# medvedevgroup/TwoPaCo

Measured on AMD Instinct MI355X. Metric: kmers_hashed_per_sec, higher is better.
Workload: dtype u64

## Files before the change

### twopaco_amd/csrc/tpc_capi.hip

```cpp
#include "tpc_ctx.h"

namespace tpch {

int fail(tpc_ctx *c, int code, const char *fmt, ...)
{
    char buf[512];
    va_list ap;
    va_start(ap, fmt);
    vsnprintf(buf, sizeof buf, fmt, ap);
    va_end(ap);
    if (c) c->err = buf;
    return code;
}





TpcLaunch make_launch(const tpc_ctx *c)
{
    TpcLaunch a;
    a.P = c->P; a.tab = c->tab; a.bases = c->bases; a.nmask = c->nmask; a.n_text = c->n_text;
    a.n_tiles = c->n_tiles; a.filter = c->filter; a.stream = c->stream;
    a.stat_kernel = c->stat_kernel;
// ... 242 lines not shown
}

extern "C" {

int tpc_ctx_create(int device, tpc_ctx **out)
{
    if (!out) return -1;
    *out = nullptr;
    int n = 0;
    if (hipGetDeviceCount(&n) != hipSuccess || n <= 0) return -2;
    if (device < 0 || device >= n) return -3;
    if (hipSetDevice(device) != hipSuccess) return -4;
    tpc_ctx *c = new tpc_ctx();
    c->device = device;
    c->dbg_ovf = getenv("TPC_DEBUG_OVF") != nullptr; c->dbg_phases = getenv("TPC_PROFILE_PHASES") != nullptr; c->dbg_timing = getenv("TWOPACO_TIMING") != nullptr; c->no_lean = TpcEnv::get().no_lean;
    if (const char *e = getenv("TPC_SHARD_TIGHT")) c->opt_shard_tight = atoi(e) ? 1 : 0;
    if (hipStreamCreate(&c->stream) != hipSuccess) { delete c; return -5; }
    for (int i = 0; i < TPC_K_COUNT; i++) {
        if (hipEventCreate(&c->ev0[i]) != hipSuccess || hipEventCreate(&c->ev1[i]) != hipSuccess) { delete c; return -5; }
    }
    if (hipMalloc((void **)&c->tab, sizeof c->tab_host) != hipSuccess ||
        hipMalloc((void **)&c->counters, 8 * sizeof(unsigned long long)) != hipSuccess ||
        hipMalloc((void **)&c->route_scratch, 128 * sizeof(unsigned long long)) != hipSuccess) { delete c; return -6; }
    *out = c;
    return 0;
}

void tpc_ctx_destroy(tpc_ctx *c)
{
    if (!c) return;
    (void)hipSetDevice(c->device);
    (void)hipStreamSynchronize(c->stream);
    void *ptrs[] = { c->tab, c->bases_alloc, c->nmask_alloc, c->filter, c->rmask, c->mask, c->marks, c->block_sums, c->table,
                     c->keys, c->idtab, c->emit_id, c->stream_buf, c->counters, c->route_scratch, c->sh_off, c->scan_blocks, c->sort_scratch, c->seg.name, c->seg.first, c->seg.ev[0], c->seg.ev[1], c->seg.ev[2],
                     c->seg.rec, c->seg.amb, c->text_plan.off, c->text_plan.piece, c->text_names, c->text_win };
    for (void *p : ptrs) if (p) (void)hipFree(p);
    stream_part_release(c);
    colors_drop(c);
    links_drop(c);
    anchors_drop(c);
    edges_drop(c);
    for (void *p : c->pbuf) if (p) (void)hipFree(p);
    for (void *p : c->ikeep) if (p) (void)hipFree(p);
    if (c->periodic) (void)hipFree(c->periodic);
    if (c->cmb_base) (void)hipFree(c->cmb_base);
    if (c->cmb_cur) (void)hipFree(c->cmb_cur);
    if (c->ikeep_ovf) (void)hipFree(c->ikeep_ovf);
    if (c->iovf_cnt) (void)hipFree(c->iovf_cnt);
    if (c->iovf_off) (void)hipFree(c->iovf_off);
    for (int i = 0; i < TPC_K_COUNT; i++) { if (c->ev0[i]) (void)hipEventDestroy(c->ev0[i]); if (c->ev1[i]) (void)hipEventDestroy(c->ev1[i]); }
    if (c->stream2) (void)hipStreamDestroy(c->stream2);
    if (c->stream) (void)hipStreamDestroy(c->stream);
    delete c;
}

const char *tpc_last_error(const tpc_ctx *c) { return c ? c->err.c_str() : "null context"; }

int tpc_set_option(tpc_ctx *c, const char *name, int64_t value)
{
    if (!c || !name) return -1;
    if (!strcmp(name, "insert_test_first")) { c->opt_test_first = value != 0; return 0; }
    if (!strcmp(name, "insert_mode")) { c->opt_insert_mode = (int)value; return 0; }
    if (!strcmp(name, "slice_bits")) { c->opt_slice_bits = (int)value; return 0; }
    if (!strcmp(name, "query_mode")) { c->opt_query_mode = (int)value; return 0; }
    if (!strcmp(name, "part_budget_bytes")) { c->opt_part_budget = value; return 0; }
    if (!strcmp(name, "part_levels")) { c->opt_part_levels = (int)value; return 0; }
    if (!strcmp(name, "shard_tight_regions")) { c->opt_shard_tight = value ? 1 : 0; c->sh_have[0] = c->sh_have[1] = false; return 0; }
    if (!strcmp(name, "part_min_tiles")) { c->opt_part_min_tiles = value < 1 ? 1 : value; return 0; }
    if (!strcmp(name, "verify_marks")) { c->opt_verify_marks = value != 0; return 0; }
    if (!strcmp(name, "mark_bucket_bits")) { tpc_test_mark_bucket_bits = (int)value; return 0; }
    if (!strcmp(name, "mark_region_cap")) { tpc_test_mark_region_cap = (int)value; return 0; }
    if (!strcmp(name, "mark_slice_bits")) { tpc_test_mark_slice_bits = (int)value; return 0; }
    if (!strcmp(name, "qhash_pushes")) { tpc_opt_qhash_pushes = value == 8 ? 8 : 6; return 0; }
    if (!strcmp(name, "qhash_roll_scalars")) { tpc_opt_qhash_roll = value != 0; return 0; }
    if (!strcmp(name, "qhash_seed_scalars")) { tpc_opt_qhash_seed = value != 0; return 0; }
    if (!strcmp(name, "fuse_apply_lookup")) { c->opt_fuse = value != 0; return 0; }
    if (!strcmp(name, "test_q6_pb2")) { tpc_test_q6_pb2 = (int)value; return 0; }
    if (!strcmp(name, "insert_entry_fmt")) { tpc_test_insert_p3 = value == 3; return 0; }
    if (!strcmp(name, "shard_periodic_skip")) { c->opt_shard_periodic = value != 0; return 0; }
    if (!strcmp(name, "periodic_skip")) { c->opt_periodic = value != 0; if (!value) c->periodic_valid = false; return 0; }
    if (!strcmp(name, "test_tight_pinch")) { tpc_test_tight_pinch = (int)value; c->sh_have[0] = c->sh_have[1] = false; return 0; }
    if (!strcmp(name, "test_sched_cap")) { tpc_test_sched_cap = value > 0 ? (uint32_t)value : 0; return 0; }
    if (!strcmp(name, "test_mask_scan")) { tpc_test_mask_scan = value == 1 || value == 2 ? (int)value : 0; return 0; }
    if (!strcmp(name, "text_window")) { c->opt_text_window = value != 0; return 0; }
    if (!strcmp(name, "replicate_filter")) { c->opt_replicate = value != 0; return 0; }
    if (!strcmp(name, "test_force_anyq")) { tpc_test_force_anyq = value != 0; return 0; }
    if (!strcmp(name, "test_sketch_grid")) { tpc_test_sketch_grid = value > 0 ? (int)value : 0; return 0; }
    if (!strcmp(name, "test_links_slots_log2")) { c->opt_links_slots_log2 = (int)std::max<int64_t>(-1, std::min<int64_t>(value, 64)); return 0; }
    if (!strcmp(name, "test_edges_slots_log2")) { c->opt_edges_slots_log2 = (int)std::max<int64_t>(-1, std::min<int64_t>(value, 64)); return 0; }
    if (!strcmp(name, "test_edges_hash_bits")) { c->opt_edges_hash_bits = (int)std::max<int64_t>(-1, std::min<int64_t>(value, 65)); return 0; }
    if (!strcmp(name, "test_locate_grid")) { c->opt_locate_grid = value > 0 ? (int)std::min<int64_t>(value, 1 << 20) : 0; return 0; }
    if (!strcmp(name, "test_distances_chunk_words")) { c->opt_distances_chunk_words = (int)std::max<int64_t>(-1, std::min<int64_t>(value, 1 << 20)); return 0; }
    if (!strcmp(name, "test_components_step_limit")) { c->opt_components_step_limit = (int)std::max<int64_t>(-1, std::min<int64_t>(value, 0x7FFFFFFF)); return 0; }
    if (!strcmp(name, "test_fail_mallocs")) { tpc_test_fail_mallocs.store(value > 0 ? (int)value : 0); return 0; }
    return fail(c, -1, "unknown option %s", name);
}

int tpc_preload(int device)
{
    if (hipSetDevice(device) != hipSuccess) { (void)hipGetLastError(); return -10; }
    const bool timing = getenv("TWOPACO_TIMING") != nullptr;
    int (*const warm[4])() = { tpc_warm_partition, tpc_warm_qpartition, tpc_warm_pass2, tpc_warm_stream };
    const char *const name[4] = { "partition", "qpartition", "pass2", "stream" };
    for (int i = 0; i < 4; i++) {
        const auto t0 = std::chrono::steady_clock::now();
        if (warm[i]() != 0) return -10;
        if (timing) fprintf(stderr, "[timing]     code object %s: %.1f ms\n", name[i], std::chrono::duration<double, std::milli>(std::chrono::steady_clock::now() - t0).count());
    }
    return 0;
}

int tpc_warmup(tpc_ctx *c)
{
    if (!c) return -1;
    return tpc_preload(c->device);
}

int64_t tpc_get_stat(const tpc_ctx *c, const char *name)
{
    if (!c || !name) return -1;
    if (!strcmp(name, "insert_path")) return c->stat_path[0];
    if (!strcmp(name, "query_path")) return c->stat_path[1];
    if (!strcmp(name, "insert_entry_fmt")) return c->stat_fmt[0];
    if (!strcmp(name, "query_entry_fmt")) return c->stat_fmt[1];
    if (!strcmp(name, "insert_hash_kernel")) return c->stat_kernel[0];
    if (!strcmp(name, "query_hash_kernel")) return c->stat_kernel[1];
    if (!strcmp(name, "query_verify_kernel")) return c->stat_kernel[2];
    if (!strcmp(name, "query_hash_form")) return c->stat_kernel[3];
    if (!strcmp(name, "query_hash_seed")) return c->stat_kernel[4];
    if (!strcmp(name, "split_kernel")) return c->stat_split[0];
    if (!strcmp(name, "split_phases")) return c->stat_split[1];
    if (!strcmp(name, "query_hash_seed_maxk")) return TPC_QSEED_MAXK;
    if (!strcmp(name, "query_mark_path")) return c->stat_mark_path;
    if (!strcmp(name, "query_mark_fallback")) return c->stat_mark_fallback;
    if (!strcmp(name, "insert_batches")) return c->stat_batches[0];
    if (!strcmp(name, "query_batches")) return c->stat_batches[1];
    if (!strcmp(name, "query_tiles_per_batch")) return c->stat_q_plan[0];
    if (!strcmp(name, "query_b1")) return c->stat_q_plan[1];
    if (!strcmp(name, "query_b2")) return c->stat_q_plan[2];
    if (!strcmp(name, "query_begun")) return c->stat_q_begun;
    if (!strcmp(name, "filter2_retries")) return c->stat_filter2_retries;
    if (!strcmp(name, "aggregate_retries")) return c->stat_aggregate_retries;
    if (!strcmp(name, "filter2_counted")) return c->stat_filter2_counted;
    if (!strcmp(name, "fused_lookups")) return c->stat_fused;
    if (!strcmp(name, "query_overflow_entries")) return c->stat_query_overflow;
    if (!strcmp(name, "insert_overflow_entries")) return c->stat_insert_overflow;
    if (!strcmp(name, "periodic_skip")) return c->periodic_valid ? 1 : 0;
    if (!strcmp(name, "pbuf_releases")) return c->stat_pbuf_releases;
    if (!strcmp(name, "distances_tile")) return TPC_DISTANCES_TILE;
    if (!strcmp(name, "text_words")) return (int64_t)(c->text_w1 - c->text_w0);
    if (!strcmp(name, "text_word_begin")) return (int64_t)c->text_w0;
    if (!strcmp(name, "text_word_end")) return (int64_t)c->text_w1;
    if (!strcmp(name, "periodic_any_query")) return c->periodic_valid && c->periodic_any_q ? 1 : 0;
    if (!strcmp(name, "periodic_any_insert")) return c->periodic_valid && c->periodic_any_i ? 1 : 0;
    if (!strcmp(name, "text_write_us")) return c->text_write_us;
    if (!strcmp(name, "text_wait_us")) return c->text_wait_us;
    if (!strcmp(name, "text_window_bytes")) return c->text_window_bytes;
    if (!strcmp(name, "device_free_bytes") || !strcmp(name, "device_total_bytes")) {
        size_t free_b = 0, total_b = 0;
        if (hipSetDevice(c->device) != hipSuccess || hipMemGetInfo(&free_b, &total_b) != hipSuccess) { (void)hipGetLastError(); return -1; }
        return (int64_t)(name[7] == 'f' ? free_b : total_b);
    }
    if (!strcmp(name, "mask_scan_form")) return tpc_stat_mask_scan_form.load(std::memory_order_relaxed);
    if (!strcmp(name, "round_marks")) return c->marks_valid ? (int64_t)c->n_marks : -1;
    return -1;
}

// ... 673 lines not shown
```

### twopaco_amd/csrc/tpc_capi_pass2.hip

```cpp
#include "tpc_ctx.h"

namespace {
int pass2_filter_impl(tpc_ctx *c, const uint64_t *fmarks, uint64_t n_fmarks, bool external, uint64_t abundance, uint64_t *n_true, uint64_t *n_false, uint64_t *table_size,
                      bool records = false, bool aggregated = false);
inline bool aggregated_counted(uint64_t abundance) { return abundance < (1ull << 40); }
}

int tpc_pass2_filter(tpc_ctx *c, uint64_t abundance, uint64_t *n_true, uint64_t *n_false, uint64_t *table_size)
{
    return pass2_filter_impl(c, nullptr, 0, false, abundance, n_true, n_false, table_size);
}

int tpc_pass2_marks(tpc_ctx *c, uint64_t *n_marks)
{
    if (!c || !c->have_params || !c->bases || !n_marks) return fail(c, -1, "set_params and seq_upload first");
    HIPCHK(c, hipSetDevice(c->device));
    int rc = compact_mask(c, c->rmask);
    if (rc) return rc;
    c->marks_valid = true;
    *n_marks = c->n_marks;
    return 0;
}

int tpc_pass2_mark_owners(tpc_ctx *c, uint32_t world, uint64_t *pos_dev, int32_t *owner_dev)
// ... 164 lines not shown
                            : tpc_launch_scan2_write(a, c->C, marks, c->table, cap, abundance, counted, c->scan_blocks, c->keys + c->n_keys * c->C))
                    return fail(c, -1, "scan2 launch failed");
                c->n_keys += tp;
            }
        }
        if (!too_full) break;
        if (cap >= full) return fail(c, -1, "exact-filter table overflow at full size");
        cap = full;
        c->stat_filter2_retries++;
    }
    if (c->rounds_done == 0) {
        HIPCHK(c, hipMemcpyAsync(c->mask, c->rmask, c->n_words_alloc * sizeof(uint32_t), hipMemcpyDeviceToDevice, c->stream));
    } else {
        tpc_launch_mask_or(c->stream, c->mask, c->rmask, c->n_words_alloc);
        c->mask_dirty = true;
    }
    c->rounds_done++;
    c->finalized = false;
    HIPCHK(c, hipGetLastError());
    HIPCHK(c, hipStreamSynchronize(c->stream));
    if (n_true) *n_true = tp;
    if (n_false) *n_false = used - tp;
    if (table_size) *table_size = used;
    return 0;
}

}

int tpc_junctions_finalize(tpc_ctx *c, uint64_t *n_junctions)
{
    if (!c || !c->have_params) return fail(c, -1, "set_params first");
    HIPCHK(c, hipSetDevice(c->device));
    {
        Timed t(c, TPC_K_SORT);
        int rc = tpc_launch_sort_keys(c->stream, c->C, c->P.k, c->keys, c->n_keys, &c->sort_scratch, &c->sort_scratch_bytes);
        if (rc) return fail(c, rc, "key sort failed (%d)", rc);
        uint64_t cap = 1024;
        while (cap < 2 * c->n_keys + 2) cap <<= 1;
        const size_t slot_bytes = c->C == 1 ? 16 : 4;
        if (cap * slot_bytes > c->idtab_bytes) {
            if (c->idtab) (void)hipFree(c->idtab);
            c->idtab = nullptr;
            c->idtab_bytes = 0;
            HIPCHK(c, dev_malloc(c, (void **)&c->idtab, cap * slot_bytes));
            c->idtab_bytes = cap * slot_bytes;
        }
        c->idtab_cap = cap;
        HIPCHK(c, hipMemsetAsync(c->idtab, 0, cap * slot_bytes, c->stream));
        if (c->n_keys >= 0xFFFFFFFFull) return fail(c, -1, "too many junctions for the 32-bit id index");
        tpc_launch_idtab_build(c->stream, c->C, c->keys, c->n_keys, c->idtab, cap);
    }
    HIPCHK(c, hipGetLastError());
    HIPCHK(c, hipStreamSynchronize(c->stream));
    c->finalized = true;
    c->keys_host.clear();
    if (n_junctions) *n_junctions = c->n_keys;
    return 0;
}

int tpc_key_words(const tpc_ctx *c) { return c ? c->C : 0; }

int tpc_junction_keys(tpc_ctx *c, uint64_t *keys_host)
{
    if (!c || !c->finalized) return fail(c, -1, "junctions_finalize first");
    HIPCHK(c, hipSetDevice(c->device));
    if (c->n_keys) HIPCHK(c, hipMemcpy(keys_host, c->keys, c->n_keys * c->C * sizeof(uint64_t), hipMemcpyDeviceToHost));
    return 0;
}

int tpc_junction_keys_raw(tpc_ctx *c, uint64_t *keys_host, uint64_t *n)
{
    if (!c || !n) return -1;
    HIPCHK(c, hipSetDevice(c->device));
    *n = c->n_keys;
    if (keys_host && c->n_keys) {
        HIPCHK(c, hipStreamSynchronize(c->stream));
        HIPCHK(c, hipMemcpy(keys_host, c->keys, c->n_keys * c->C * sizeof(uint64_t), hipMemcpyDeviceToHost));
    }
    return 0;
}

int tpc_junction_keys_set(tpc_ctx *c, const uint64_t *keys_host, uint64_t n)
{
// ... 305 lines not shown
```

### twopaco_amd/csrc/tpc_ctx.h

```cpp
#pragma once
#include "../../include/twopaco_hip.h"
#include "tpc_internal.h"

#include <algorithm>
#include <atomic>
#include <cmath>
#include <chrono>
#include <cstdarg>
#include <cstdio>
#include <cstdlib>
#include <cstring>
#include <string>
#include <vector>
#include <map>

struct tpc_ctx {
    __attribute__((always_inline)) tpc_ctx() = default;
    int device = 0;
    hipStream_t stream = nullptr;
    std::string err;
    bool have_params = false;
    TpcHashParams P{};
    uint64_t tab_host[TPC_TAB_WORDS + TPC_QSEED_WORDS]{};
    uint64_t *tab = nullptr;
// ... 5 lines not shown
    uint32_t *periodic = nullptr;
    bool periodic_valid = false;
    bool periodic_any_q = false, periodic_any_i = false;
    int opt_periodic = 1;
    bool opt_shard_periodic = false;
    uint64_t *bases_alloc = nullptr;
    uint32_t *nmask_alloc = nullptr;
    int opt_text_window = 0;
    bool text_windowed = false;
    uint64_t text_w0 = 0, text_w1 = 0;
    uint32_t *filter = nullptr;
    uint64_t filter_words = 0;
    uint32_t *rmask = nullptr, *mask = nullptr;
    bool mask_dirty = false;
    int rounds_done = 0;
    uint64_t *marks = nullptr;
    uint64_t marks_cap = 0, n_marks = 0;
    bool marks_valid = false;
    bool rmask_sums_valid = false;
    uint64_t rmask_sums_n = 0;
    uint64_t *block_sums = nullptr;
    uint64_t *scan_blocks = nullptr;
    void *table = nullptr;
    uint64_t table_cap = 0, table_alloc = 0;
    uint64_t *keys = nullptr;
    uint64_t n_keys = 0, keys_cap = 0;
    bool finalized = false;
    std::vector<uint64_t> keys_host;
    uint32_t *idtab = nullptr;
    uint64_t idtab_cap = 0;
    size_t idtab_bytes = 0;
    void *sort_scratch = nullptr;
    size_t sort_scratch_bytes = 0;
    int64_t *emit_id = nullptr;
    uint64_t emit_cap = 0, n_emit = 0;
    uint32_t *stream_buf = nullptr;
    uint64_t stream_cap = 0, stream_bytes = 0;
    uint64_t *sp_rec = nullptr, *sp_vscan = nullptr, *sp_cnt = nullptr, *sp_lo = nullptr;
    uint32_t *sp_flags = nullptr;
    uint32_t sp_n_rec = 0;
    struct Segments {
        int64_t *name = nullptr;
        uint32_t *first = nullptr;
        uint32_t *ev[3] = {nullptr, nullptr, nullptr};
        uint32_t n_rec = 0;
        uint64_t events = 0, segments = 0, named = 0, table_bytes = 0, slots = 0, peak_bytes = 0;
        uint64_t err_slot = 0;
        int err_kind = 0;
        bool valid = false;
        uint64_t *rec = nullptr, *amb = nullptr;
        uint64_t n_amb = 0, text_n = 0, text_uploads = 0;
        const void *text_bases = nullptr;
        int k = 0;
    } seg;
    TpcTextPlan text_plan;
    void *text_names = nullptr;
    uint8_t *text_win = nullptr;
    size_t text_win_cap = 0;
    bool text_valid = false;
    uint64_t text_total = 0;
    double text_ms = 0;
    int64_t text_write_us = 0, text_wait_us = 0, text_window_bytes = 0;
    struct Colors {
        uint32_t *rows = nullptr;
        uint32_t *presence = nullptr;
        unsigned long long *hist = nullptr;
// ... 65 lines not shown
        unsigned long long *shared = nullptr;
        uint64_t positions = 0, windows = 0, found = 0, n_runs = 0, n_rec = 0, peak_bytes = 0;
        uint32_t n_colors = 0;
        bool valid = false;
    } loc;
    int opt_edges_slots_log2 = 0;
    int opt_edges_hash_bits = 0;
    int opt_locate_grid = 0;
    int opt_components_step_limit = 0;
    int opt_distances_chunk_words = 0;
    unsigned long long *counters = nullptr;
    unsigned long long *route_scratch = nullptr;
    uint64_t *sh_off = nullptr;
    size_t sh_off_bytes = 0;
    int opt_test_first = 0;
    int opt_insert_mode = 0;
    int opt_slice_bits = 20;
    bool filter_zero_pending = false;
    static constexpr int NPBUF = 19;
    void *pbuf[NPBUF] = {};
    size_t pbytes[NPBUF] = {};
    std::vector<uint64_t> off2_uploaded, off3_uploaded;
    int opt_part_levels = 0;
    int opt_shard_tight = 1;
    int stat_path[2] = {0, 0};
    int64_t stat_batches[2] = {0, 0};
    mutable int stat_kernel[5] = {0, 0, 0, 0, 0};
    mutable int stat_split[2] = {0, 0};
    int stat_fmt[2] = {0, 0};
    int64_t stat_filter2_retries = 0;
    int64_t stat_aggregate_retries = 0;
    int stat_filter2_counted = 0;
    int opt_verify_marks = 1;
    int stat_mark_path = 0;
    int64_t stat_mark_fallback = 0;
    int64_t opt_part_min_tiles = 256;
    int64_t opt_part_budget = 0;
    int opt_query_mode = 0;
    int opt_fuse = 1;
    bool pending_apply = false;
    bool pending_fresh = false;
    bool pending_shard = false;
    TpcPartPlan pending_pl;
    void *ikeep[2] = {nullptr, nullptr};
    size_t ikeep_bytes[2] = {0, 0};
    uint64_t *ikeep_ovf = nullptr;
    uint64_t ikeep_ovf_cap = 0;
    uint64_t pending_novf = 0;
    uint32_t *iovf_cnt = nullptr;
    uint64_t *iovf_off = nullptr;
    uint32_t iovf_slices = 0;
    int64_t stat_fused = 0;
    int64_t stat_query_overflow = 0;
    int64_t stat_insert_overflow = 0;
    int64_t stat_pbuf_releases = 0;
    uint32_t sh_rank = 0, sh_world = 1;
    TpcPartPlan sh_ipl;
    TpcQPlan sh_qpl;
    bool sh_have[2] = {false, false};
    uint64_t sh_per[2] = {0, 0}, sh_batches[2] = {0, 0};
    uint64_t sh_nsurv = 0;
    bool sh_defer = false;
    bool sh_ovf_set[2] = {false, false};
    hipStream_t stream2 = nullptr;
    bool sh_async[2] = {false, false};
    unsigned long long sh_ov_host[2][2] = {{0, 0}, {0, 0}};
// ... 86 lines not shown
```

### twopaco_amd/csrc/tpc_internal.h

```cpp
#pragma once
#include "tpc_device.h"
#include <algorithm>
#include <atomic>
#include <cstdlib>
#include <vector>

struct TpcEnv {
    bool no_lean, rb_hash, verify_eager, gated_full;
    int verify_marks;
    int qhash_pushes, qhash_roll, qhash_seed;
    int ppr_insert, gated_loads, split_loads9;
    int slice_grid;
    static const TpcEnv &get()
    {
        static const TpcEnv e = [] {
            TpcEnv v;
            v.no_lean = getenv("TPC_NO_LEAN") != nullptr;
            v.rb_hash = getenv("TPC_RB_HASH") != nullptr;
            const char *lz = getenv("TPC_VERIFY_LAZY");
            v.verify_eager = lz && lz[0] == '0';
            v.gated_full = getenv("TPC_GATED_FULL_REGIONS") != nullptr;
            const char *vm = getenv("TPC_VERIFY_MARKS");
            v.verify_marks = vm && vm[0] ? (vm[0] != '0' ? 1 : 0) : -1;
            const char *qp = getenv("TPC_QHASH_PUSHES");
            v.qhash_pushes = qp && (atoi(qp) == 6 || atoi(qp) == 8) ? atoi(qp) : 0;
            const char *qr = getenv("TPC_QHASH_ROLL_SCALARS");
            v.qhash_roll = qr && qr[0] ? (qr[0] != '0' ? 1 : 0) : -1;
            const char *qs = getenv("TPC_QHASH_SEED_SCALARS");
            v.qhash_seed = qs && qs[0] ? (qs[0] != '0' ? 1 : 0) : -1;
            const char *p = getenv("TPC_PPR_INSERT"), *g = getenv("TPC_GATED_LOADS");
            v.ppr_insert = p ? atoi(p) : 0;
            v.gated_loads = g ? atoi(g) : 0;
            const char *s9 = getenv("TPC_SPLIT_LOADS9");
            v.split_loads9 = s9 ? atoi(s9) : 0;
            const char *lg = getenv("TPC_LOOKUP_GRID");
            int n_cu = 0, dev = 0;
            if (hipGetDevice(&dev) != hipSuccess || hipDeviceGetAttribute(&n_cu, hipDeviceAttributeMultiprocessorCount, dev) != hipSuccess || n_cu <= 0) { (void)hipGetLastError(); n_cu = 256; }
            v.slice_grid = lg ? atoi(lg) : 2 * n_cu;
            return v;
        }();
        return e;
    }
};

inline uint32_t tpc_slice_grid(uint32_t n_slices)
{
    const int g = TpcEnv::get().slice_grid;
    return g > 0 ? std::min<uint32_t>(n_slices, (uint32_t)g) : n_slices;
}

extern int tpc_opt_qhash_pushes, tpc_opt_qhash_roll, tpc_opt_qhash_seed;
inline bool tpc_qhash_roll_scalars() { const int e = TpcEnv::get().qhash_roll; return (e >= 0 ? e : tpc_opt_qhash_roll) != 0; }
inline bool tpc_qhash_seed_scalars() { const int e = TpcEnv::get().qhash_seed; return (e >= 0 ? e : tpc_opt_qhash_seed) != 0; }
inline bool tpc_qhash_compact() { const int e = TpcEnv::get().qhash_pushes; return (e ? e : tpc_opt_qhash_pushes) != 8; }

#define TPC_TAB_MAXQ 64
// ... 171 lines not shown

struct TpcCombineOut { uint16_t *payload; uint64_t cap; unsigned long long *cur; uint64_t *dir; uint32_t n_dest; };
constexpr uint32_t TPC_COMBINE_PERSIST_SLICES = 16384, TPC_COMBINE_CHUNK = 512, TPC_COMBINE_MAX_WG = 1024;
int tpc_launch_slice_combine(const TpcLaunch &a, int slice_bits, int b1, int b2, uint32_t perm_mult, uint32_t perm_inv, const TpcPartPlan *ipl, const uint64_t *iovf,
                             const uint64_t *iovf_off, const TpcListSrc &ls, bool dense, bool fresh, const TpcCombineOut *out, uint32_t rank, uint32_t world);

int tpc_launch_mask_count(hipStream_t s, const uint32_t *mask, uint64_t n_words, uint64_t *block_sums, unsigned long long *n_out);
extern int tpc_test_mask_scan;
extern std::atomic<int> tpc_stat_mask_scan_form;
int tpc_launch_mask_scatter(hipStream_t s, const uint32_t *mask, uint64_t n_words, const uint64_t *block_sums, uint64_t *list);
int tpc_launch_mask_or(hipStream_t s, uint32_t *dst, const uint32_t *src, uint64_t n_words);

size_t tpc_table_slot_bytes(int C);
int tpc_launch_table_init(hipStream_t s, void *table, uint64_t cap);
#define TPC_FILTER2_PROBE_LIMIT 512u
int tpc_launch_mark_owner(const TpcLaunch &a, int C, const uint64_t *marks, uint64_t n_marks, uint32_t world, int32_t *owner);
int tpc_launch_mark_records(const TpcLaunch &a, int C, const uint64_t *marks, uint64_t n_marks, uint32_t world, uint64_t *records, int32_t *owner);
int tpc_launch_table_records(const TpcLaunch &a, int C, const uint64_t *marks, const void *table, uint64_t cap, const uint64_t *block_off, uint32_t world,
                             uint64_t *records, int32_t *owner);
int tpc_launch_filter2_rec(const TpcLaunch &a, int C, const uint64_t *records, uint64_t n, void *table, uint64_t cap, bool counted, unsigned long long *overflow);
int tpc_launch_scan2_write_rec(const TpcLaunch &a, int C, const uint64_t *records, const void *table, uint64_t cap, uint64_t abundance, bool counted,
                               const uint64_t *block_off, uint64_t *keys_out);
int tpc_launch_permute_rows(hipStream_t s, const uint64_t *src, const uint32_t *perm, uint64_t n, int row_words, uint64_t *dst);
int tpc_launch_filter2(const TpcLaunch &a, int C, const uint64_t *marks, uint64_t n_marks, void *table, uint64_t cap, bool counted,
                       unsigned long long *overflow);
#define TPC_SCAN2_BLOCKS 4096
int tpc_launch_scan2_count(const TpcLaunch &a, const void *table, uint64_t cap, uint64_t abundance, bool counted, uint64_t *block_tp,
                           uint64_t *block_used, unsigned long long *totals);
int tpc_launch_scan2_write(const TpcLaunch &a, int C, const uint64_t *marks, const void *table, uint64_t cap, uint64_t abundance, bool counted,
                           const uint64_t *block_off, uint64_t *keys_out);

int tpc_launch_sort_keys(hipStream_t s, int C, int k, uint64_t *keys, uint64_t J, void **scratch, size_t *scratch_bytes);

int tpc_launch_idtab_build(hipStream_t s, int C, const uint64_t *keys, uint64_t J, uint32_t *idtab, uint64_t cap);
int tpc_launch_emit(const TpcLaunch &a, int C, const uint64_t *marks, uint64_t n_marks, const uint64_t *keys, uint64_t J,
                    const uint32_t *idtab, uint64_t cap, int64_t *ids, unsigned long long *n_valid);

size_t tpc_stream_plan_bytes(uint32_t n_rec);
int tpc_launch_stream_plan(hipStream_t s, const uint64_t *d_rec_start, const uint64_t *d_rec_len, uint32_t n_rec, int k, const uint64_t *marks,
                           const int64_t *ids, uint64_t n_marks, uint64_t *vscan, void *rec, uint32_t r_last, uint64_t *totals_host);
int tpc_launch_stream_write(hipStream_t s, const uint64_t *d_rec_start, const uint64_t *d_rec_len, uint32_t n_rec, int k, const uint64_t *marks,
                            const int64_t *ids, uint64_t n_marks, const uint64_t *vscan, const void *rec, uint32_t r_last, uint64_t first_stub, uint32_t *out);

int tpc_launch_stream_partial(hipStream_t s, const uint64_t *d_rec_start, const uint64_t *d_rec_len, uint32_t n_rec, int k, const uint64_t *marks,
                              const int64_t *ids, uint64_t n_marks, uint64_t *vscan, uint64_t *cnt, uint32_t *flags, uint64_t *mark_lo);
int tpc_launch_stream_write_part(hipStream_t s, const uint64_t *d_rec_start, const uint64_t *d_rec_len, uint32_t n_rec, int k, const uint64_t *marks,
                                 const int64_t *ids, uint64_t n_marks, const uint64_t *vscan, const uint64_t *mark_lo, const uint32_t *gflags,
                                 const uint64_t *e_scan, const uint64_t *s_scan, const uint64_t *before, uint32_t r_last, uint64_t first_stub,
                                 uint64_t chunk_lo, uint64_t chunk_hi, uint64_t slot0, uint32_t *out);

int tpc_warm_pass1();
int tpc_warm_partition();
int tpc_warm_qpartition();
int tpc_warm_pass2();
int tpc_warm_stream();
extern int tpc_test_sketch_grid;
#define TPC_SEG_ERR_TEXT 256
struct TpcSegResult { uint64_t events, segments, named, table_bytes, peak_bytes, err_slot; int err_kind; };
int tpc_launch_segments(hipStream_t s, const uint32_t *slots, uint64_t n_slots, int k, const uint64_t *bases, const uint32_t *nmask,
                        const uint64_t *d_rec_start, const uint64_t *d_rec_len, uint32_t n_rec, const uint64_t *d_amb, uint64_t n_amb,
                        int64_t **name_out, uint32_t **first_out, uint32_t **ev_out , TpcSegResult *res, char *err);
struct TpcTextPlan {
    int format = 0, k = 0;
    uint64_t n_events = 0;
    uint32_t n_rec = 0;
    const int64_t *name = nullptr;
// ... 16 lines not shown
```

### twopaco_amd/csrc/tpc_pass2.hip

```cpp
#include "tpc_device.h"
#include "tpc_internal.h"
#include <rocprim/rocprim.hpp>
#include <algorithm>

#ifndef TPC_PASS2_PART
#define TPC_PASS2_PART 0
#endif
#if TPC_PASS2_PART == 0
#define TPC_PASS2_FN(name) name
#else
#define TPC_PASS2_FN(name) name##_long
#endif

namespace {

constexpr uint64_t EMPTY = ~0ull;
constexpr int META_NEXT_SHIFT = 5;
constexpr int META_COUNT_SHIFT = 16;
constexpr uint64_t META_MULTI = 1ull << 10;

struct Slot { uint64_t key; uint64_t meta; };

__device__ __forceinline__ uint32_t wave_incl_scan(uint32_t v)
{
// ... 581 lines not shown
                }
                if (keys_equal<C>(sk, ck)) {
                    id = keys_equal<C>(ck, fw) ? (int64_t)r : -(int64_t)r;
                    valid++;
                    break;
                }
                slot = (slot + 1) & mask;
            }
        }
        ids[idx] = id;
    }
    block_add64(n_valid, valid, s_w);
}

__global__ void k_iota(uint32_t *p, uint64_t n)
{
    const uint64_t i = (uint64_t)blockIdx.x * blockDim.x + threadIdx.x;
    if (i < n) p[i] = (uint32_t)i;
}
__global__ void k_gather_word(const uint64_t *__restrict__ keys, const uint32_t *__restrict__ perm, uint64_t n, int C, int w, uint64_t *out)
{
    const uint64_t i = (uint64_t)blockIdx.x * blockDim.x + threadIdx.x;
    if (i < n) out[i] = keys[(uint64_t)perm[i] * C + w];
}
__global__ void k_gather_keys(const uint64_t *__restrict__ keys, const uint32_t *__restrict__ perm, uint64_t n, int C, uint64_t *out)
{
    const uint64_t i = (uint64_t)blockIdx.x * blockDim.x + threadIdx.x;
    if (i < n)
        for (int w = 0; w < C; w++) out[i * C + w] = keys[(uint64_t)perm[i] * C + w];
}

inline unsigned nblk(uint64_t n, unsigned b) { return (unsigned)((n + b - 1) / b); }

}

#if TPC_PASS2_PART == 0
#define TPC_DISPATCH_C(C_, CALL)                                                                  \
    switch (C_) {                                                                                 \
    case 1: CALL(1); break; case 2: CALL(2); break;                                               \
    default: return -1;                                                                           \
    }
#else
#define TPC_DISPATCH_C(C_, CALL)                                                                  \
    switch (C_) {                                                                                 \
    case 3: CALL(3); break; case 4: CALL(4); break;                                               \
    case 5: CALL(5); break; case 6: CALL(6); break; case 7: CALL(7); break; case 8: CALL(8); break;       \
    case 9: CALL(9); break; case 10: CALL(10); break; case 11: CALL(11); break; case 12: CALL(12); break; \
    case 13: CALL(13); break; case 14: CALL(14); break; case 15: CALL(15); break; case 16: CALL(16); break; \
    case 17: CALL(17); break; case 18: CALL(18); break; case 19: CALL(19); break;                 \
    default: return -1;                                                                           \
    }
#endif
int tpc_launch_filter2_long(const TpcLaunch &a, int C, const uint64_t *marks, uint64_t n_marks, void *table, uint64_t cap, bool counted,
                            unsigned long long *overflow);
int tpc_launch_scan2_write_long(const TpcLaunch &a, int C, const uint64_t *marks, const void *table, uint64_t cap, uint64_t abundance, bool counted,
                                const uint64_t *block_off, uint64_t *keys_out);
int tpc_launch_idtab_build_long(hipStream_t s, int C, const uint64_t *keys, uint64_t J, uint32_t *idtab, uint64_t cap);
int tpc_launch_sort_keys_long(hipStream_t s, int C, uint64_t *keys, uint64_t J);
int tpc_launch_emit_long(const TpcLaunch &a, int C, const uint64_t *marks, uint64_t n_marks, const uint64_t *keys, uint64_t J,
                         const uint32_t *idtab, uint64_t cap, int64_t *ids, unsigned long long *n_valid);

#if TPC_PASS2_PART == 0
constexpr uint32_t SCAN_SEG = 4096;
__global__ void __launch_bounds__(256) k_scan_sums_seg(const uint64_t *__restrict__ block_sums, uint64_t n, unsigned long long *__restrict__ seg_tot)
{
    __shared__ unsigned long long s64[4];
// ... 186 lines not shown
#define CALL(C_) hipLaunchKernelGGL((k_scan2_write<C_>), dim3(TPC_SCAN2_BLOCKS), dim3(256), 0, a.stream, a.P, a.tab, a.bases, marks, (const Slot *)table, cap, chunk, abundance, counted ? 1 : 0, block_off, keys_out)
    TPC_DISPATCH_C(C, CALL)
#undef CALL
    return 0;
}

#if TPC_PASS2_PART == 0
int tpc_launch_sort_keys(hipStream_t s, int C, int k, uint64_t *keys, uint64_t J, void **scratch, size_t *scratch_bytes)
{
    if (J < 2) return 0;
    hipError_t e;
    if (C == 1) {
        size_t tmp_bytes = 0;
        int end_bit = 2 * k;
        if (end_bit > 64) end_bit = 64;
        uint64_t *out = nullptr;
        if ((e = rocprim::radix_sort_keys(nullptr, tmp_bytes, keys, out, J, 0, end_bit, s)) != hipSuccess) return -2;
        const size_t out_bytes = (J * sizeof(uint64_t) + 255) & ~(size_t)255;
        const size_t need = out_bytes + (tmp_bytes ? tmp_bytes : 8);
        if (need > *scratch_bytes) {
            if (*scratch) (void)hipFree(*scratch);
            *scratch = nullptr; *scratch_bytes = 0;
            if (hipMalloc(scratch, need + need / 4) != hipSuccess) return -3;
            *scratch_bytes = need + need / 4;
        }
        out = (uint64_t *)*scratch;
        void *tmp = (char *)*scratch + out_bytes;
        e = rocprim::radix_sort_keys(tmp, tmp_bytes, keys, out, J, 0, end_bit, s);
        if (e == hipSuccess) e = hipMemcpyAsync(keys, out, J * sizeof(uint64_t), hipMemcpyDeviceToDevice, s);
        return e == hipSuccess ? 0 : -2;
    }
    return tpc_launch_sort_keys_long(s, C, keys, J);
}
#endif

#if TPC_PASS2_PART == 1
int tpc_launch_sort_keys_long(hipStream_t s, int C, uint64_t *keys, uint64_t J)
{
    uint64_t *kw = nullptr, *kw2 = nullptr, *out = nullptr;
    uint32_t *perm = nullptr, *perm2 = nullptr;
    void *tmp = nullptr;
    size_t tmp_bytes = 0;
    int rc = 0;
    if (rocprim::radix_sort_pairs(nullptr, tmp_bytes, kw, kw2, perm, perm2, J, 0, 64, s) != hipSuccess) return -2;
    if (hipMalloc(&kw, J * 8) != hipSuccess || hipMalloc(&kw2, J * 8) != hipSuccess || hipMalloc(&out, J * C * 8) != hipSuccess ||
        hipMalloc(&perm, J * 4) != hipSuccess || hipMalloc(&perm2, J * 4) != hipSuccess || hipMalloc(&tmp, tmp_bytes ? tmp_bytes : 8) != hipSuccess) {
        rc = -3;
    } else {
        hipLaunchKernelGGL(k_iota, dim3(nblk(J, 256)), dim3(256), 0, s, perm, J);
        for (int w = C - 1; w >= 0 && rc == 0; w--) {
            hipLaunchKernelGGL(k_gather_word, dim3(nblk(J, 256)), dim3(256), 0, s, keys, perm, J, C, w, kw);
            if (rocprim::radix_sort_pairs(tmp, tmp_bytes, kw, kw2, perm, perm2, J, 0, 64, s) != hipSuccess) rc = -2;
            uint32_t *t = perm; perm = perm2; perm2 = t;
        }
        if (rc == 0) {
            hipLaunchKernelGGL(k_gather_keys, dim3(nblk(J, 256)), dim3(256), 0, s, keys, perm, J, C, out);
            if (hipMemcpyAsync(keys, out, J * C * 8, hipMemcpyDeviceToDevice, s) != hipSuccess) rc = -2;
        }
        (void)hipStreamSynchronize(s);
    }
    (void)hipFree(kw); (void)hipFree(kw2); (void)hipFree(out); (void)hipFree(perm); (void)hipFree(perm2); (void)hipFree(tmp);
    return rc;
}
#endif

int TPC_PASS2_FN(tpc_launch_idtab_build)(hipStream_t s, int C, const uint64_t *keys, uint64_t J, uint32_t *idtab, uint64_t cap)
// ... 29 lines not shown
```

Baseline: 12.85 billion.

## Replace radix key sort with bucketed top-bit sort fused with id-table build

For single-word keys, the junction key sort is replaced by a histogram, scan and scatter on the top key bits, followed by a per-bucket bitonic sort in LDS. That per-bucket kernel also inserts each sorted key into the id hash table. The aim is to avoid the multi-pass rocprim radix sort, the device copy and the separate idtab build kernel. If any bucket exceeds the LDS cap, the code syncs to read the max bucket size and falls back to the radix path, which costs an extra host round trip.

```diff
diff --git a/twopaco_amd/csrc/tpc_capi.hip b/twopaco_amd/csrc/tpc_capi.hip
--- a/twopaco_amd/csrc/tpc_capi.hip
+++ b/twopaco_amd/csrc/tpc_capi.hip
@@ -298,7 +298,7 @@
     (void)hipSetDevice(c->device);
     (void)hipStreamSynchronize(c->stream);
     void *ptrs[] = { c->tab, c->bases_alloc, c->nmask_alloc, c->filter, c->rmask, c->mask, c->marks, c->block_sums, c->table,
-                     c->keys, c->idtab, c->emit_id, c->stream_buf, c->counters, c->route_scratch, c->sh_off, c->scan_blocks, c->sort_scratch, c->seg.name, c->seg.first, c->seg.ev[0], c->seg.ev[1], c->seg.ev[2],
+                     c->keys, c->idtab, c->emit_id, c->stream_buf, c->counters, c->route_scratch, c->sh_off, c->scan_blocks, c->sort_scratch, c->ksort_hdr, c->seg.name, c->seg.first, c->seg.ev[0], c->seg.ev[1], c->seg.ev[2],
                      c->seg.rec, c->seg.amb, c->text_plan.off, c->text_plan.piece, c->text_names, c->text_win };
     for (void *p : ptrs) if (p) (void)hipFree(p);
     stream_part_release(c);
@@ -334,6 +334,7 @@
     if (!strcmp(name, "shard_tight_regions")) { c->opt_shard_tight = value ? 1 : 0; c->sh_have[0] = c->sh_have[1] = false; return 0; }
     if (!strcmp(name, "part_min_tiles")) { c->opt_part_min_tiles = value < 1 ? 1 : value; return 0; }
     if (!strcmp(name, "verify_marks")) { c->opt_verify_marks = value != 0; return 0; }
+    if (!strcmp(name, "key_sort")) { c->opt_key_sort = value != 0; return 0; }
     if (!strcmp(name, "mark_bucket_bits")) { tpc_test_mark_bucket_bits = (int)value; return 0; }
     if (!strcmp(name, "mark_region_cap")) { tpc_test_mark_region_cap = (int)value; return 0; }
     if (!strcmp(name, "mark_slice_bits")) { tpc_test_mark_slice_bits = (int)value; return 0; }
@@ -399,6 +400,10 @@
     if (!strcmp(name, "query_hash_seed_maxk")) return TPC_QSEED_MAXK;
     if (!strcmp(name, "query_mark_path")) return c->stat_mark_path;
     if (!strcmp(name, "query_mark_fallback")) return c->stat_mark_fallback;
+    if (!strcmp(name, "key_sort_form")) return c->stat_key_sort[0];
+    if (!strcmp(name, "key_sort_bits")) return c->stat_key_sort[1];
+    if (!strcmp(name, "key_sort_cap")) return TPC_KEY_SORT_CAP;
+    if (!strcmp(name, "key_sort_max_bits")) return TPC_KEY_SORT_MAX_BITS;
     if (!strcmp(name, "insert_batches")) return c->stat_batches[0];
     if (!strcmp(name, "query_batches")) return c->stat_batches[1];
     if (!strcmp(name, "query_tiles_per_batch")) return c->stat_q_plan[0];
diff --git a/twopaco_amd/csrc/tpc_capi_pass2.hip b/twopaco_amd/csrc/tpc_capi_pass2.hip
--- a/twopaco_amd/csrc/tpc_capi_pass2.hip
+++ b/twopaco_amd/csrc/tpc_capi_pass2.hip
@@ -220,9 +220,17 @@
     if (!c || !c->have_params) return fail(c, -1, "set_params first");
     HIPCHK(c, hipSetDevice(c->device));
     {
-        Timed t(c, TPC_K_SORT);
-        int rc = tpc_launch_sort_keys(c->stream, c->C, c->P.k, c->keys, c->n_keys, &c->sort_scratch, &c->sort_scratch_bytes);
-        if (rc) return fail(c, rc, "key sort failed (%d)", rc);
+        if (c->n_keys >= 0xFFFFFFFFull) return fail(c, -1, "too many junctions for the 32-bit id index");
+        const int env_sort = TpcEnv::get().key_sort;
+        bool buckets = c->C == 1 && c->n_keys >= 2 && (env_sort >= 0 ? env_sort != 0 : c->opt_key_sort != 0);
+        if (buckets && !c->ksort_hdr) {
+            HIPCHK(c, dev_malloc(c, (void **)&c->ksort_hdr, TPC_KEY_SORT_HDR_WORDS * sizeof(uint32_t)));
+            HIPCHK(c, hipMemsetAsync(c->ksort_hdr, 0, TPC_KEY_SORT_HDR_WORDS * sizeof(uint32_t), c->stream));
+        }
+        c->stat_key_sort[0] = c->n_keys < 2 ? 0 : 1;
+        c->stat_key_sort[1] = 0;
+        (void)hipEventRecord(c->ev0[TPC_K_SORT], c->stream);
+        c->ev_used[TPC_K_SORT] = true;
         uint64_t cap = 1024;
         while (cap < 2 * c->n_keys + 2) cap <<= 1;
         const size_t slot_bytes = c->C == 1 ? 16 : 4;
@@ -235,8 +243,26 @@
         }
         c->idtab_cap = cap;
         HIPCHK(c, hipMemsetAsync(c->idtab, 0, cap * slot_bytes, c->stream));
-        if (c->n_keys >= 0xFFFFFFFFull) return fail(c, -1, "too many junctions for the 32-bit id index");
-        tpc_launch_idtab_build(c->stream, c->C, c->keys, c->n_keys, c->idtab, cap);
+        if (buckets) {
+            int bits = 0;
+            int rc = tpc_launch_sort_keys_buckets(c->stream, c->P.k, c->keys, c->n_keys, &c->sort_scratch, &c->sort_scratch_bytes, c->ksort_hdr, c->idtab, cap, &bits);
+            if (rc) return fail(c, rc, "key sort failed (%d)", rc);
+            (void)hipEventRecord(c->ev1[TPC_K_SORT], c->stream);
+            c->stat_key_sort[0] = 2;
+            c->stat_key_sort[1] = bits;
+            if (bits > 0) {
+                uint32_t largest = 0;
+                HIPCHK(c, hipMemcpyAsync(&largest, c->ksort_hdr + TPC_KEY_SORT_HDR_MAX, sizeof largest, hipMemcpyDeviceToHost, c->stream));
+                HIPCHK(c, hipStreamSynchronize(c->stream));
+                if (largest > TPC_KEY_SORT_CAP) { buckets = false; c->stat_key_sort[0] = 3; }
+            }
+        }
+        if (!buckets) {
+            int rc = tpc_launch_sort_keys(c->stream, c->C, c->P.k, c->keys, c->n_keys, &c->sort_scratch, &c->sort_scratch_bytes);
+            if (rc) return fail(c, rc, "key sort failed (%d)", rc);
+            tpc_launch_idtab_build(c->stream, c->C, c->keys, c->n_keys, c->idtab, cap);
+            (void)hipEventRecord(c->ev1[TPC_K_SORT], c->stream);
+        }
     }
     HIPCHK(c, hipGetLastError());
     HIPCHK(c, hipStreamSynchronize(c->stream));
diff --git a/twopaco_amd/csrc/tpc_ctx.h b/twopaco_amd/csrc/tpc_ctx.h
--- a/twopaco_amd/csrc/tpc_ctx.h
+++ b/twopaco_amd/csrc/tpc_ctx.h
@@ -61,6 +61,7 @@
     size_t idtab_bytes = 0;
     void *sort_scratch = nullptr;
     size_t sort_scratch_bytes = 0;
+    uint32_t *ksort_hdr = nullptr;
     int64_t *emit_id = nullptr;
     uint64_t emit_cap = 0, n_emit = 0;
     uint32_t *stream_buf = nullptr;
@@ -192,6 +193,8 @@
     int64_t stat_aggregate_retries = 0;
     int stat_filter2_counted = 0;
     int opt_verify_marks = 1;
+    int opt_key_sort = 1;
+    int stat_key_sort[2] = {0, 0};
     int stat_mark_path = 0;
     int64_t stat_mark_fallback = 0;
     int64_t opt_part_min_tiles = 256;
diff --git a/twopaco_amd/csrc/tpc_internal.h b/twopaco_amd/csrc/tpc_internal.h
--- a/twopaco_amd/csrc/tpc_internal.h
+++ b/twopaco_amd/csrc/tpc_internal.h
@@ -8,6 +8,7 @@
 struct TpcEnv {
     bool no_lean, rb_hash, verify_eager, gated_full;
     int verify_marks;
+    int key_sort;
     int qhash_pushes, qhash_roll, qhash_seed;
     int ppr_insert, gated_loads, split_loads9;
     int slice_grid;
@@ -22,6 +23,8 @@
             v.gated_full = getenv("TPC_GATED_FULL_REGIONS") != nullptr;
             const char *vm = getenv("TPC_VERIFY_MARKS");
             v.verify_marks = vm && vm[0] ? (vm[0] != '0' ? 1 : 0) : -1;
+            const char *ks = getenv("TPC_KEY_SORT");
+            v.key_sort = ks && ks[0] ? (ks[0] != '0' ? 1 : 0) : -1;
             const char *qp = getenv("TPC_QHASH_PUSHES");
             v.qhash_pushes = qp && (atoi(qp) == 6 || atoi(qp) == 8) ? atoi(qp) : 0;
             const char *qr = getenv("TPC_QHASH_ROLL_SCALARS");
@@ -259,6 +262,14 @@
 
 int tpc_launch_sort_keys(hipStream_t s, int C, int k, uint64_t *keys, uint64_t J, void **scratch, size_t *scratch_bytes);
 
+#define TPC_KEY_SORT_CAP 1024
+#define TPC_KEY_SORT_MAX_BITS 11
+#define TPC_KEY_SORT_HDR_WORDS 8192
+#define TPC_KEY_SORT_HDR_MAX (3 * (1 << TPC_KEY_SORT_MAX_BITS) + 1)
+int tpc_key_sort_bits(int k, uint64_t J);
+int tpc_launch_sort_keys_buckets(hipStream_t s, int k, uint64_t *keys, uint64_t J, void **scratch, size_t *scratch_bytes, uint32_t *hdr,
+                                 uint32_t *idtab, uint64_t cap, int *bits);
+
 int tpc_launch_idtab_build(hipStream_t s, int C, const uint64_t *keys, uint64_t J, uint32_t *idtab, uint64_t cap);
 int tpc_launch_emit(const TpcLaunch &a, int C, const uint64_t *marks, uint64_t n_marks, const uint64_t *keys, uint64_t J,
                     const uint32_t *idtab, uint64_t cap, int64_t *ids, unsigned long long *n_valid);
diff --git a/twopaco_amd/csrc/tpc_pass2.hip b/twopaco_amd/csrc/tpc_pass2.hip
--- a/twopaco_amd/csrc/tpc_pass2.hip
+++ b/twopaco_amd/csrc/tpc_pass2.hip
@@ -637,6 +637,140 @@
 
 inline unsigned nblk(uint64_t n, unsigned b) { return (unsigned)((n + b - 1) / b); }
 
+#if TPC_PASS2_PART == 0
+constexpr uint32_t KS_CAP = TPC_KEY_SORT_CAP;
+constexpr uint32_t KS_MAXB = 1u << TPC_KEY_SORT_MAX_BITS;
+constexpr uint32_t KS_COUNT = 0;
+constexpr uint32_t KS_OFF = KS_MAXB;
+constexpr uint32_t KS_CUR = 2 * KS_MAXB + 1;
+constexpr uint32_t KS_MAX = 3 * KS_MAXB + 1;
+constexpr uint32_t KS_CHUNK = 8192;
+constexpr int KS_LOADS = 8;
+static_assert(KS_MAX < TPC_KEY_SORT_HDR_WORDS, "key sort header");
+
+__device__ __forceinline__ uint32_t ksort_bucket(uint64_t key, int shift, uint32_t nb)
+{
+    const uint64_t b = key >> shift;
+    return b < nb ? (uint32_t)b : nb - 1;
+}
+
+__device__ __forceinline__ void ksort_count_chunk(const uint64_t *__restrict__ keys, uint64_t i0, uint64_t i1, int shift, uint32_t nb, uint32_t *s_h)
+{
+    for (uint32_t b = threadIdx.x; b < nb; b += 256) s_h[b] = 0;
+    __syncthreads();
+    for (uint64_t base = i0 + threadIdx.x; base < i1; base += 256 * KS_LOADS) {
+        uint64_t key[KS_LOADS];
+#pragma unroll
+        for (int j = 0; j < KS_LOADS; j++) key[j] = base + 256 * j < i1 ? keys[base + 256 * j] : 0;
+#pragma unroll
+        for (int j = 0; j < KS_LOADS; j++)
+            if (base + 256 * j < i1) atomicAdd(&s_h[ksort_bucket(key[j], shift, nb)], 1u);
+    }
+    __syncthreads();
+}
+
+__global__ void __launch_bounds__(256) k_ksort_hist(const uint64_t *__restrict__ keys, uint64_t J, int shift, uint32_t nb, uint32_t *hdr)
+{
+    __shared__ uint32_t s_h[KS_MAXB];
+    const uint64_t i0 = (uint64_t)blockIdx.x * KS_CHUNK, i1 = min(J, i0 + KS_CHUNK);
+    ksort_count_chunk(keys, i0, i1, shift, nb, s_h);
+    for (uint32_t b = threadIdx.x; b < nb; b += 256)
+        if (s_h[b]) atomicAdd(&hdr[KS_COUNT + b], s_h[b]);
+}
+
+__global__ void __launch_bounds__(256) k_ksort_scan(uint32_t nb, uint64_t J, uint32_t *hdr)
+{
+    __shared__ uint32_t s_w[4], s_m[4];
+    constexpr uint32_t PER = KS_MAXB / 256;
+    uint32_t v[PER], sum = 0, mx = 0;
+#pragma unroll
+    for (uint32_t j = 0; j < PER; j++) {
+        const uint32_t b = threadIdx.x * PER + j;
+        v[j] = b < nb ? hdr[KS_COUNT + b] : 0;
+        if (b < nb) hdr[KS_COUNT + b] = 0;
+        sum += v[j];
+        mx = max(mx, v[j]);
+    }
+    uint32_t total;
+    uint32_t run = block_excl_scan256(sum, s_w, total);
+#pragma unroll
+    for (uint32_t j = 0; j < PER; j++) {
+        const uint32_t b = threadIdx.x * PER + j;
+        if (b < nb) { hdr[KS_OFF + b] = run; hdr[KS_CUR + b] = run; }
+        run += v[j];
+    }
+    for (int o = 32; o > 0; o >>= 1) mx = max(mx, (uint32_t)__shfl_xor(mx, o, 64));
+    if ((threadIdx.x & 63) == 0) s_m[threadIdx.x >> 6] = mx;
+    __syncthreads();
+    if (threadIdx.x == 0) {
+        hdr[KS_OFF + nb] = (uint32_t)J;
+        hdr[KS_MAX] = max(max(s_m[0], s_m[1]), max(s_m[2], s_m[3]));
+    }
+}
+
+__global__ void __launch_bounds__(256) k_ksort_scatter(const uint64_t *__restrict__ keys, uint64_t J, int shift, uint32_t nb, uint32_t *hdr,
+                                                       uint64_t *__restrict__ out)
+{
+    __shared__ uint32_t s_h[KS_MAXB];
+    if (hdr[KS_MAX] > KS_CAP) return;
+    const uint64_t i0 = (uint64_t)blockIdx.x * KS_CHUNK, i1 = min(J, i0 + KS_CHUNK);
+    ksort_count_chunk(keys, i0, i1, shift, nb, s_h);
+    for (uint32_t b = threadIdx.x; b < nb; b += 256) {
+        const uint32_t n = s_h[b];
+        if (n) s_h[b] = atomicAdd(&hdr[KS_CUR + b], n);
+    }
+    __syncthreads();
+    for (uint64_t base = i0 + threadIdx.x; base < i1; base += 256 * KS_LOADS) {
+        uint64_t key[KS_LOADS];
+#pragma unroll
+        for (int j = 0; j < KS_LOADS; j++) key[j] = base + 256 * j < i1 ? keys[base + 256 * j] : 0;
+#pragma unroll
+        for (int j = 0; j < KS_LOADS; j++) {
+            if (base + 256 * j >= i1) continue;
+            const uint32_t pos = atomicAdd(&s_h[ksort_bucket(key[j], shift, nb)], 1u);
+            if (pos < J) out[pos] = key[j];
+        }
+    }
+}
+
+__global__ void __launch_bounds__(256) k_ksort_local(const uint64_t *src, uint64_t *keys, uint64_t J, uint32_t nb,
+                                                     const uint32_t *__restrict__ hdr, uint32_t *idtab, uint64_t cap)
+{
+    __shared__ uint64_t s_k[KS_CAP];
+    if (hdr && hdr[KS_MAX] > KS_CAP) return;
+    const uint64_t mask = cap - 1;
+    for (uint32_t b = blockIdx.x; b < nb; b += gridDim.x) {
+        const uint32_t o0 = hdr ? hdr[KS_OFF + b] : 0u, o1 = hdr ? hdr[KS_OFF + b + 1] : (uint32_t)J;
+        const uint32_t n = o1 - o0;
+        if (n == 0 || n > KS_CAP || o1 > J) continue;
+        uint32_t p2 = 1;
+        while (p2 < n) p2 <<= 1;
+        for (uint32_t i = threadIdx.x; i < p2; i += 256) s_k[i] = i < n ? src[o0 + i] : ~0ull;
+        __syncthreads();
+        for (uint32_t size = 2; size <= p2; size <<= 1)
+            for (uint32_t j = size >> 1; j > 0; j >>= 1) {
+                for (uint32_t t = threadIdx.x; t < (p2 >> 1); t += 256) {
+                    const uint32_t lo = ((t & ~(j - 1)) << 1) | (t & (j - 1)), hi = lo | j;
+                    const uint64_t x = s_k[lo], y = s_k[hi];
+                    if ((x > y) == ((lo & size) == 0)) { s_k[lo] = y; s_k[hi] = x; }
+                }
+                __syncthreads();
+            }
+        for (uint32_t i = threadIdx.x; i < n; i += 256) {
+            const uint64_t key = s_k[i];
+            keys[o0 + i] = key;
+            if (idtab) {
+                const uint64_t kk[1] = {key};
+                uint64_t slot = key_hash<1>(kk) & mask;
+                while (atomicCAS(&idtab[slot * 4 + 2], 0u, o0 + i + 1) != 0u) slot = (slot + 1) & mask;
+                *reinterpret_cast<uint64_t *>(idtab + slot * 4) = key;
+            }
+        }
+        __syncthreads();
+    }
+}
+#endif
+
 }
 
 #if TPC_PASS2_PART == 0
@@ -889,6 +1023,40 @@
     }
     return tpc_launch_sort_keys_long(s, C, keys, J);
 }
+
+int tpc_key_sort_bits(int k, uint64_t J)
+{
+    if (J <= KS_CAP) return 0;
+    int B = 1;
+    while ((J >> B) > KS_CAP / 4 && B < TPC_KEY_SORT_MAX_BITS) B++;
+    return std::min(B, 2 * k);
+}
+
+int tpc_launch_sort_keys_buckets(hipStream_t s, int k, uint64_t *keys, uint64_t J, void **scratch, size_t *scratch_bytes, uint32_t *hdr,
+                                 uint32_t *idtab, uint64_t cap, int *bits)
+{
+    if (J < 2 || J >= 0xFFFFFFFFull || !hdr || !bits) return -1;
+    const int B = *bits = tpc_key_sort_bits(k, J);
+    if (B == 0) {
+        hipLaunchKernelGGL(k_ksort_local, dim3(1), dim3(256), 0, s, (const uint64_t *)keys, keys, J, 1u, (const uint32_t *)nullptr, idtab, cap);
+        return 0;
+    }
+    const size_t need = J * sizeof(uint64_t);
+    if (need > *scratch_bytes) {
+        if (*scratch) (void)hipFree(*scratch);
+        *scratch = nullptr; *scratch_bytes = 0;
+        if (hipMalloc(scratch, need + need / 4) != hipSuccess) return -3;
+        *scratch_bytes = need + need / 4;
+    }
+    const int shift = 2 * k - B;
+    const uint32_t nb = 1u << B;
+    const unsigned grid = nblk(J, KS_CHUNK);
+    hipLaunchKernelGGL(k_ksort_hist, dim3(grid), dim3(256), 0, s, (const uint64_t *)keys, J, shift, nb, hdr);
+    hipLaunchKernelGGL(k_ksort_scan, dim3(1), dim3(256), 0, s, nb, J, hdr);
+    hipLaunchKernelGGL(k_ksort_scatter, dim3(grid), dim3(256), 0, s, (const uint64_t *)keys, J, shift, nb, hdr, (uint64_t *)*scratch);
+    hipLaunchKernelGGL(k_ksort_local, dim3(nb), dim3(256), 0, s, (const uint64_t *)*scratch, keys, J, nb, (const uint32_t *)hdr, idtab, cap);
+    return 0;
+}
 #endif
 
 #if TPC_PASS2_PART == 1
```

New measurement: 12.90 billion (median of 6 runs). About the same (+0.4%).
